# AuroraEchos/Sound-Event-Localization-and-Detection

Hardware: AMD Instinct MI355X
Metric: train-step samples/sec (8ch x 128mel x 512T) (higher is better)
Workload: dtype f32; 1 GPU; c3: DQSELD-TCN-S1-PHI_8ch train step, F=128 T=512 (U=L=192, SURVEY F3), batch 32/GPU, random-init weights; global_batch=32, parallelism=dp1, step_mode=graph (auto: probe 9.51 ms recorded / 10.23 ms eager per step), deterministic=True

## Files before the change

### sound-event-localization-and-detection_amd/csrc/first_stage.hip

```cpp
#include <string.h>
#include <type_traits>
#include "hc_common.h"

namespace seld {

constexpr int FS_K = 72;
constexpr int FS_KP = 80;
constexpr int FS_WEXT = 72, FS_DPAD = 4;
constexpr int FS_XR = 10;
constexpr int FS_NTILE = 15;

typedef unsigned int uintx4f __attribute__((ext_vector_type(4)));

__host__ __device__ constexpr int fs_tri(int t, int u) { return t * 5 - t * (t - 1) / 2 + (u - t); }

constexpr int FS_XI = (8 * FS_XR * (FS_WEXT / 4) + 255) / 256;
__device__ __forceinline__ void fs_load_x(const float* x, uintx4f (&v)[FS_XI], int n, int h0, int w0, int H, int W, int tid) {
    const unsigned S = (unsigned)(H * W);
    const unsigned OOB = 0xFFFFFFF0u;
    const __amdgpu_buffer_rsrc_t rsrc = __builtin_amdgcn_make_buffer_rsrc((void*)(x + (size_t)n * 8 * S), 0, 8u * S * 4u, 0x00020000);
    constexpr int qw = FS_WEXT / 4;
#pragma unroll
    for (int i = 0; i < FS_XI; ++i) {
        const int f = tid + 256 * i;
        const int row = f / qw, quad = f - row * qw;
        const int ch = row / FS_XR, xr = row - ch * FS_XR;
        const int hh = h0 - 1 + xr, ww = w0 - FS_DPAD + 4 * quad;
        const bool ok = f < 8 * FS_XR * qw && (unsigned)hh < (unsigned)H && (unsigned)ww < (unsigned)W;
        const unsigned e = ((unsigned)ch * (unsigned)H + (unsigned)hh) * (unsigned)W + (unsigned)ww;
        v[i] = __builtin_amdgcn_raw_buffer_load_b128(rsrc, ok ? e * 4u : OOB, 0, 0);
    }
}
__device__ __forceinline__ void fs_store_x(float* lds, const uintx4f (&v)[FS_XI], int tid) {
#pragma unroll
    for (int i = 0; i < FS_XI; ++i) {
        const int f = tid + 256 * i;
        if (f < 8 * FS_XR * (FS_WEXT / 4))
            *reinterpret_cast<float4*>(lds + f * 4) =
                make_float4(__uint_as_float(v[i][0]), __uint_as_float(v[i][1]), __uint_as_float(v[i][2]), __uint_as_float(v[i][3]));
    }
}
struct FsGramP {
    const float* x;
    float* part;
    int N, H, W;
    int nblocks;
};

__global__ __launch_bounds__(256, 2) void fs_gram_kernel(const FsGramP p) {
    __shared__ __attribute__((aligned(16))) float lds[8 * FS_XR * FS_WEXT > 3 * FS_NTILE * 256 ? 8 * FS_XR * FS_WEXT : 3 * FS_NTILE * 256];
    const int tid = threadIdx.x, lane = tid & 63;
    const int wave = __builtin_amdgcn_readfirstlane(tid >> 6);
    const int fr = lane & 15, fk = lane >> 4;
    int goff[5];
    float gone[5];
    bool gld[5];
#pragma unroll
    for (int t = 0; t < 5; ++t) {
        const int kk = 16 * t + fr;
        const int kc = kk < FS_K ? kk : 0;
        const int ch = kc / 9, tap = kc - ch * 9, kh = tap / 3, kw = tap - kh * 3;
        goff[t] = (ch * FS_XR + kh) * FS_WEXT + FS_DPAD + 16 * wave + fk + (kw - 1);
        gld[t] = kk < FS_K;
        gone[t] = kk == FS_K ? 1.f : 0.f;
    }
    floatx4 acc[FS_NTILE];
#pragma unroll
    for (int i = 0; i < FS_NTILE; ++i) acc[i] = (floatx4){0.f, 0.f, 0.f, 0.f};

    const int wq = p.W >> 6, hq = p.H >> 3;
    uintx4f xv[FS_XI];
    auto request = [&](int b) __attribute__((always_inline)) {
        const int n = b / (hq * wq), rem = b - n * (hq * wq);
        fs_load_x(p.x, xv, n, (rem / wq) * 8, (rem % wq) * 64, p.H, p.W, tid);
    };
    if ((int)blockIdx.x < p.nblocks) request(blockIdx.x);
    for (int b = blockIdx.x; b < p.nblocks; b += gridDim.x) {
        __syncthreads();
        fs_store_x(lds, xv, tid);
        __syncthreads();
        if (b + (int)gridDim.x < p.nblocks) request(b + gridDim.x);
        __builtin_amdgcn_sched_barrier(0);
#pragma unroll 1
        for (int r = 0; r < 8; ++r) {
#pragma unroll
            for (int j = 0; j < 4; ++j) {
                float v[5];
#pragma unroll
                for (int t = 0; t < 5; ++t) v[t] = gld[t] ? lds[goff[t] + r * FS_WEXT + 4 * j] : gone[t];
#pragma unroll
                for (int t = 0; t < 5; ++t)
#pragma unroll
                    for (int u = t; u < 5; ++u)
                        acc[fs_tri(t, u)] = __builtin_amdgcn_mfma_f32_16x16x4f32(v[t], v[u], acc[fs_tri(t, u)], 0, 0, 0);
            }
        }
    }
    __syncthreads();
    if (wave > 0) {
        float* dst = lds + (wave - 1) * FS_NTILE * 256 + lane * 4;
#pragma unroll
        for (int i = 0; i < FS_NTILE; ++i) *reinterpret_cast<floatx4*>(dst + i * 256) = acc[i];
    }
    __syncthreads();
    if (wave == 0) {
        float* out = p.part + (size_t)blockIdx.x * FS_NTILE * 256 + lane * 4;
#pragma unroll
        for (int i = 0; i < FS_NTILE; ++i) {
            floatx4 a = acc[i];
#pragma unroll
            for (int w = 0; w < 3; ++w) a += *reinterpret_cast<const floatx4*>(lds + w * FS_NTILE * 256 + i * 256 + lane * 4);
            *reinterpret_cast<floatx4*>(out + i * 256) = a;
        }
    }
}

__global__ __launch_bounds__(256) void fs_sum_parts_kernel(const float* __restrict__ part, int nparts, int n, double* __restrict__ red) {
    __shared__ double sh[4][64];
    const int lane = threadIdx.x & 63, wave = threadIdx.x >> 6;
    const int e = blockIdx.x * 64 + lane;
    double a = 0.0;
    if (e < n) {
        int w = wave;
        for (; w + 28 < nparts; w += 32) {
            float v[8];
#pragma unroll
            for (int k = 0; k < 8; ++k) v[k] = part[(size_t)(w + 4 * k) * n + e];
#pragma unroll
            for (int k = 0; k < 8; ++k) a += (double)v[k];
        }
        for (; w < nparts; w += 4) a += (double)part[(size_t)w * n + e];
    }
    sh[wave][lane] = a;
    __syncthreads();
    if (wave == 0 && e < n) red[e] = ((sh[0][lane] + sh[1][lane]) + sh[2][lane]) + sh[3][lane];
}
__global__ __launch_bounds__(256) void fs_gram_fold_kernel(const double* __restrict__ tiles, double* __restrict__ gram) {
    const int e = blockIdx.x * 256 + threadIdx.x;
    if (e >= FS_KP * FS_KP) return;
    const int i = e / FS_KP, j = e - i * FS_KP;
    const int lo = i < j ? i : j, hi = i < j ? j : i;
    const int t = lo >> 4, u = hi >> 4;
    int row, col;
    if (t == u) { row = i & 15; col = j & 15; }
    else { row = lo & 15; col = hi & 15; }
    const int ln = (row >> 2) * 16 + col;
    gram[e] = tiles[(size_t)fs_tri(t, u) * 256 + ln * 4 + (row & 3)];
}

struct FsW {
    const float* w[8];
    int A, OB, IB;
};
__device__ __forceinline__ float fs_wfull(const FsW& f, int c, int kk) {
    const int ch = kk / 9, tap = kk - ch * 9;
    const int po = c / f.OB, ob = c - po * f.OB;
    const int qi = ch / f.IB, ib = ch - qi * f.IB;
    float sign;
    const int comp = block_comp(f.A, po, qi, &sign);
    if (comp < 0) return 0.f;
    return sign * f.w[comp][((size_t)ob * f.IB + ib) * 9 + tap];
}

struct FsBnP {
    FsW w;
    const double* gram;
    const float* bias;
    float* mean;
    float* invstd;
    float* rmean;
    float* rvar;
    long long* nbt;
    float* wg;
    int C;
    float eps, momentum;
};
__global__ __launch_bounds__(256) void fs_bn_from_gram_kernel(const FsBnP p) {
    __shared__ double wrow[FS_K];
    __shared__ double red1[4], red2[4];
    const int c = blockIdx.x, tid = threadIdx.x;
    if (tid < FS_K) wrow[tid] = (double)fs_wfull(p.w, c, tid);
    __syncthreads();
    double m2 = 0.0, m1 = 0.0;
    if (tid < FS_K) {
        double row = 0.0;
        for (int k = 0; k < FS_K; ++k) row += wrow[k] * p.gram[tid * FS_KP + k];
        if (p.wg) p.wg[(size_t)c * FS_K + tid] = (float)row;
        m2 = wrow[tid] * row;
        m1 = wrow[tid] * p.gram[FS_K * FS_KP + tid];
    }
#pragma unroll
    for (int o = 32; o > 0; o >>= 1) {
        m1 += __shfl_xor(m1, o, 64);
        m2 += __shfl_xor(m2, o, 64);
    }
    if ((tid & 63) == 0) { red1[tid >> 6] = m1; red2[tid >> 6] = m2; }
    __syncthreads();
    if (tid != 0) return;
    if (c == 0 && p.nbt) *p.nbt += 1;
    const double count = p.gram[FS_K * FS_KP + FS_K];
    const double t1 = (red1[0] + red1[1] + red1[2] + red1[3]) / count;
    double var = (red2[0] + red2[1] + red2[2] + red2[3]) / count - t1 * t1;
    if (var < 0.0) var = 0.0;
    const double m = t1 + (p.bias ? (double)p.bias[c] : 0.0);
    p.mean[c] = (float)m;
    p.invstd[c] = (float)(1.0 / sqrt(var + (double)p.eps));
    if (p.rmean) p.rmean[c] = (1.f - p.momentum) * p.rmean[c] + p.momentum * (float)m;
    if (p.rvar) {
        const double unbiased = count > 1.0 ? var * count / (count - 1.0) : var;
        p.rvar[c] = (1.f - p.momentum) * p.rvar[c] + p.momentum * (float)unbiased;
    }
}

struct FsRedP {
    const float* dout;
    const float* out;
    const float* raw;
    const float* mean;
    const float* invstd;
    const float* gamma;
    const float* beta;
    float* part;
    int N, C, S;
    int nchunk;
    float scale;
};
__global__ __launch_bounds__(256) void fs_reduce_kernel(const FsRedP p) {
    const int c = blockIdx.y, chunk = blockIdx.x;
    const float mu = p.mean[c], is = p.invstd[c];
    const float ga = p.gamma[c], be = p.beta[c];
    const bool degenerate = ga == 0.f;
    const float inv_g = degenerate ? 0.f : 1.0f / ga, inv_scale = 1.0f / p.scale;
    const long long total = (long long)p.N * p.S;
    const long long per = ((total / 4 + p.nchunk - 1) / p.nchunk) * 4;
    const long long beg = (long long)chunk * per;
    long long end = beg + per;
    if (end > total) end = total;
    float v0 = 0.f, v1 = 0.f;
    for (long long k = beg + threadIdx.x * 4; k < end; k += 256 * 4) {
        const long long n = k / p.S;
        const size_t off = ((size_t)n * p.C + c) * p.S + (size_t)(k - n * p.S);
        float4 r4 = make_float4(0.f, 0.f, 0.f, 0.f);
        if (degenerate) r4 = *reinterpret_cast<const float4*>(p.raw + off);
        const float4 d4 = *reinterpret_cast<const float4*>(p.dout + off);
        const float4 o4 = *reinterpret_cast<const float4*>(p.out + off);
        const float rr[4] = {r4.x, r4.y, r4.z, r4.w}, dd[4] = {d4.x, d4.y, d4.z, d4.w}, oo[4] = {o4.x, o4.y, o4.z, o4.w};
#pragma unroll
        for (int e = 0; e < 4; ++e)
            if (oo[e] != 0.f) {
                const float dz = dd[e] * p.scale;
                v0 += dz * (degenerate ? (rr[e] - mu) * is : (oo[e] * inv_scale - be) * inv_g);
                v1 += dz;
            }
    }
    __shared__ float r0[4], r1[4];
    v0 = wave_sum(v0);
    v1 = wave_sum(v1);
    if ((threadIdx.x & 63) == 0) { r0[threadIdx.x >> 6] = v0; r1[threadIdx.x >> 6] = v1; }
    __syncthreads();
    if (threadIdx.x == 0) {
        float* o = p.part + ((size_t)c * p.nchunk + chunk) * 2;
        o[0] = (r0[0] + r0[1]) + (r0[2] + r0[3]);
        o[1] = (r1[0] + r1[1]) + (r1[2] + r1[3]);
    }
}
__global__ void fs_coef_kernel(const float* __restrict__ part, int nchunk, const float* __restrict__ mean,
                               const float* __restrict__ invstd, const float* __restrict__ gamma, int C, double count,
                               float* __restrict__ dgamma, float* __restrict__ dbeta, float* __restrict__ coef) {
    const int c = blockIdx.x * blockDim.x + threadIdx.x;
    if (c >= C) return;
    double s0 = 0.0, s1 = 0.0;
    for (int k = 0; k < nchunk; ++k) {
        s0 += (double)part[((size_t)c * nchunk + k) * 2];
        s1 += (double)part[((size_t)c * nchunk + k) * 2 + 1];
    }
    dgamma[c] += (float)s0;
    dbeta[c] += (float)s1;
    const float mu = mean[c], is = invstd[c], a = gamma[c] * is;
    const float k1 = (float)(s1 / count), k2 = (float)(s0 / count);
    coef[c] = -a * is * k2;
    coef[C + c] = a;
    coef[2 * C + c] = a * (mu * is * k2 - k1);
}

struct FsWgP {
    const float* x;
    const float* dout;
    const float* out;
    const unsigned char* idx;
    const float* invstd;
    const float* gamma;
    float* part;
    int N, C, H, W;
    int nblocks;
    float scale;
};

template <int NTW, bool DQ>
__global__ __launch_bounds__(512, 2) void fs_wgrad_kernel(const FsWgP p) {
    constexpr int NARROW = DQ ? NTW / 2 : 0;
    constexpr int NACC = NARROW * 3 + (NTW - NARROW) * 5;
    constexpr int XT = 8 * FS_XR * FS_WEXT;
    constexpr int RED = 2 * NACC * 256;
    __shared__ __attribute__((aligned(16))) float lds[(2 * XT > RED ? 2 * XT : RED) + 192];
    const int tid = threadIdx.x, lane = tid & 63;
    const int wave = __builtin_amdgcn_readfirstlane(tid >> 6);
    const int hc = wave >> 2, cq = wave & 3;
    const int fr = lane & 15, fk = lane >> 4;
    int goff[5];
    bool gld[5];
#pragma unroll
    for (int t = 0; t < 5; ++t) {
        const int kk = 16 * t + fr;
        const int kc = kk < FS_K ? kk : 0;
        const int ch = kc / 9, tap = kc - ch * 9, kh = tap / 3, kw = tap - kh * 3;
        goff[t] = (ch * FS_XR + kh) * FS_WEXT + FS_DPAD + 16 * cq + fk + (kw - 1);
        gld[t] = kk < FS_K;
    }
    auto ctile = [&](int i) __attribute__((always_inline)) -> int {
        if (DQ) return i < NARROW ? hc * NARROW + i : NTW + hc * NARROW + (i - NARROW);
        return hc * NTW + i;
    };
    float* const ab = lds + 2 * XT;
    for (int c = tid; c < p.C; c += 512) ab[c] = p.gamma[c] * p.invstd[c] * p.scale;
    auto acc_idx = [](int i, int u) constexpr { return i < NARROW ? i * 3 + u : NARROW * 3 + (i - NARROW) * 5 + u; };
    floatx4 acc[NACC];
#pragma unroll
    for (int i = 0; i < NACC; ++i) acc[i] = (floatx4){0.f, 0.f, 0.f, 0.f};

    const int wq = p.W >> 6, hq = p.H >> 3, PH = hq;
    const size_t PS = (size_t)PH * p.W;
    constexpr int QW = FS_WEXT / 4, NQ = 8 * FS_XR * QW, NST = (NQ + 511) / 512;
    float4 stage[NST];
    auto fetch_tile = [&](int b) __attribute__((always_inline)) {
        const int n = b / (hq * wq), rem = b - n * (hq * wq);
        const int h0 = (rem / wq) * 8, w0 = (rem % wq) * 64;
#pragma unroll
        for (int k = 0; k < NST; ++k) {
            const int f = tid + 512 * k;
            const int row = f / QW, quad = f - row * QW;
            const int ch = row / FS_XR, xr = row - ch * FS_XR;
            const int hh = h0 - 1 + xr, ww = w0 - FS_DPAD + 4 * quad;
            stage[k] = make_float4(0.f, 0.f, 0.f, 0.f);
            if (f < NQ && (unsigned)hh < (unsigned)p.H && (unsigned)ww < (unsigned)p.W)
                stage[k] = *reinterpret_cast<const float4*>(p.x + (((size_t)n * 8 + ch) * p.H + hh) * p.W + ww);
        }
    };
    auto store_tile = [&](float* buf) __attribute__((always_inline)) {
#pragma unroll
        for (int k = 0; k < NST; ++k) {
            const int f = tid + 512 * k;
            if (f < NQ) *reinterpret_cast<float4*>(buf + f * 4) = stage[k];
        }
    };
    float vz[NTW];
    unsigned rpk = 0;
    float ld_o[NTW], ld_d[NTW];
    unsigned ld_i[NTW];
    auto issue_group = [&](int b, int jg) __attribute__((always_inline)) {
        const int n = b / (hq * wq), rem = b - n * (hq * wq);
        const int q = rem / wq, w0 = (rem % wq) * 64;
#pragma unroll
        for (int i = 0; i < NTW; ++i) {
            const int chn = ctile(i) * 16 + fr;
            const size_t off = ((size_t)n * p.C + chn) * PS + (size_t)q * p.W + (size_t)(w0 + 16 * cq + 4 * jg + fk);
            ld_o[i] = p.out[off];
            ld_d[i] = p.dout[off];
            ld_i[i] = p.idx[off];
        }
    };
    auto finish_group = [&]() __attribute__((always_inline)) {
        unsigned pk = 0;
#pragma unroll
        for (int i = 0; i < NTW; ++i) {
            const float a_ = ab[ctile(i) * 16 + fr];
            vz[i] = ld_o[i] != 0.f ? ld_d[i] * a_ : 0.f;
            pk |= (ld_i[i] & 7u) << (3 * i);
        }
        rpk = pk;
    };
    int bufsel = 0;
    if ((int)blockIdx.x < p.nblocks) { fetch_tile(blockIdx.x); store_tile(lds); }
    __syncthreads();
    if ((int)blockIdx.x < p.nblocks) issue_group(blockIdx.x, 0);
    for (int b = blockIdx.x; b < p.nblocks; b += gridDim.x) {
        const float* xt = lds + bufsel * XT;
        const bool more = b + (int)gridDim.x < p.nblocks;
        if (more) fetch_tile(b + gridDim.x);
        float bv[5], bn_[5];
#pragma unroll
        for (int u = 0; u < 5; ++u) bv[u] = gld[u] ? xt[goff[u]] : 0.f;
#pragma unroll
        for (int jg = 0; jg < 4; ++jg) {
            finish_group();
            if (jg + 1 < 4) issue_group(b, jg + 1);
            else if (more) issue_group(b + gridDim.x, 0);
#pragma unroll 2
            for (int r = 0; r < 8; ++r) {
                const int rn = r + 1 < 8 ? r + 1 : 0, jn = r + 1 < 8 ? jg : (jg + 1 < 4 ? jg + 1 : 0);
#pragma unroll
                for (int u = 0; u < 5; ++u) bn_[u] = gld[u] ? xt[goff[u] + rn * FS_WEXT + 4 * jn] : 0.f;
#pragma unroll
                for (int i = 0; i < NTW; ++i) {
                    const float av = ((rpk >> (3 * i)) & 7u) == (unsigned)r ? vz[i] : 0.f;
#pragma unroll
                    for (int u = 0; u < (i < NARROW ? 3 : 5); ++u)
                        acc[acc_idx(i, u)] = __builtin_amdgcn_mfma_f32_16x16x4f32(av, bv[u], acc[acc_idx(i, u)], 0, 0, 0);
                }
#pragma unroll
                for (int u = 0; u < 5; ++u) bv[u] = bn_[u];
            }
        }
        if (more) store_tile(lds + (bufsel ^ 1) * XT);
        bufsel ^= 1;
        __syncthreads();
    }
#pragma unroll 1
    for (int k = 1; k < 4; ++k) {
        __syncthreads();
        if (cq == k) {
            float* dst = lds + hc * NACC * 256 + lane * 4;
#pragma unroll
            for (int i = 0; i < NACC; ++i) *reinterpret_cast<floatx4*>(dst + i * 256) = acc[i];
        }
        __syncthreads();
        if (cq == 0) {
            const float* src = lds + hc * NACC * 256 + lane * 4;
#pragma unroll
            for (int i = 0; i < NACC; ++i) acc[i] += *reinterpret_cast<const floatx4*>(src + i * 256);
        }
    }
    if (cq == 0) {
        float* out = p.part + (size_t)blockIdx.x * (2 * NTW) * 5 * 256 + lane * 4;
#pragma unroll
        for (int i = 0; i < NTW; ++i)
#pragma unroll
            for (int u = 0; u < 5; ++u) {
                floatx4 v = (floatx4){0.f, 0.f, 0.f, 0.f};
                if (u < (i < NARROW ? 3 : 5)) v = acc[acc_idx(i, u)];
                *reinterpret_cast<floatx4*>(out + (ctile(i) * 5 + u) * 256) = v;
            }
    }
}

struct FsWsumP {
    const double* sum;
    const float* wg;
    const double* gram;
    const float* coef;
    const float* bias;
    float* dwf;
    int C;
};
__global__ __launch_bounds__(256) void fs_wsum_kernel(const FsWsumP p) {
    const int e = blockIdx.x * 256 + threadIdx.x;
    if (e >= p.C * FS_K) return;
    const int c = e / FS_K, kk = e - c * FS_K;
    const int ct = c >> 4, row = c & 15, u = kk >> 4, col = kk & 15;
    double a = p.sum[((size_t)ct * 5 + u) * 256 + ((row >> 2) * 16 + col) * 4 + (row & 3)];
    const double sk = p.gram[FS_K * FS_KP + kk];
    a += (double)p.coef[c] * ((double)p.wg[e] + (p.bias ? (double)p.bias[c] * sk : 0.0)) + (double)p.coef[2 * p.C + c] * sk;
    p.dwf[e] = (float)a;
}
struct FsWfoldP {
    const float* dwf;
    float* dw[8];
    int A, OB, IB, C;
};
__global__ __launch_bounds__(256) void fs_wfold_kernel(const FsWfoldP p) {
    const int per = p.OB * p.IB * 9;
    const int e = blockIdx.x * 256 + threadIdx.x;
    if (e >= p.A * per) return;
    const int comp = e / per;
    int rem = e - comp * per;
    const int ob = rem / (p.IB * 9);
    rem -= ob * p.IB * 9;
    const int ib = rem / 9, tap = rem - ib * 9;
    float a = 0.f;
    for (int po = 0; po < p.A; ++po)
        for (int qi = 0; qi < p.A; ++qi) {
            float sign;
            if (block_comp(p.A, po, qi, &sign) != comp) continue;
            a += sign * p.dwf[(size_t)(po * p.OB + ob) * FS_K + (qi * p.IB + ib) * 9 + tap];
        }
    p.dw[comp][((size_t)ob * p.IB + ib) * 9 + tap] += a;
}

static int fs_shape_ok(const seld_conv_desc* d) {
    if (hc_validate(d) != SELD_OK) return 0;
    if (d->ndim != 2 || d->Cin != 8 || d->k[0] != 3 || d->k[1] != 3) return 0;
    if (d->stride[0] != 1 || d->stride[1] != 1 || d->dil[0] != 1 || d->dil[1] != 1 || d->pad[0] != 1 || d->pad[1] != 1) return 0;
    if (d->in[0] % 8 || d->in[1] % 64) return 0;
    if ((long long)d->N * d->Cout * d->in[0] * d->in[1] * 4 >= (1LL << 32)) return 0;
    return 1;
}
static int fs_gram_wgs(const seld_conv_desc* d) {
    const long long nblocks = (long long)d->N * (d->in[0] / 8) * (d->in[1] / 64);
    return (int)(nblocks < 512 ? nblocks : 512);
}

}
using namespace seld;

extern "C" size_t seld_first_stage_gram_workspace(const seld_conv_desc* d) {
    if (!fs_shape_ok(d)) return 0;
    return (size_t)FS_KP * FS_KP * sizeof(double) + (size_t)FS_NTILE * 256 * sizeof(double) +
           (size_t)fs_gram_wgs(d) * FS_NTILE * 256 * sizeof(float);
}

extern "C" int seld_first_stage_gram(const seld_conv_desc* d, const float* x, void* workspace, size_t workspace_bytes, void* stream) {
    if (!d || !x || !workspace) return SELD_EINVAL;
    const size_t need = seld_first_stage_gram_workspace(d);
    if (!need) return SELD_EUNSUPPORTED;
    if (workspace_bytes < need || ((uintptr_t)workspace & 15)) return SELD_EWORKSPACE;
    FsGramP p{};
    p.x = x; p.N = d->N; p.H = d->in[0]; p.W = d->in[1];
    p.nblocks = d->N * (d->in[0] / 8) * (d->in[1] / 64);
    double* gram = (double*)workspace;
    double* tiles = gram + FS_KP * FS_KP;
    p.part = (float*)(tiles + FS_NTILE * 256);
    const int nwg = fs_gram_wgs(d);
    hipStream_t st = (hipStream_t)stream;
    hipLaunchKernelGGL(fs_gram_kernel, dim3(nwg), dim3(256), 0, st, p);
    int rc = check_launch();
    if (rc) return rc;
    hipLaunchKernelGGL(fs_sum_parts_kernel, dim3(FS_NTILE * 256 / 64), dim3(256), 0, st, p.part, nwg, FS_NTILE * 256, tiles);
    rc = check_launch();
    if (rc) return rc;
    hipLaunchKernelGGL(fs_gram_fold_kernel, dim3((FS_KP * FS_KP + 255) / 256), dim3(256), 0, st, tiles, gram);
    return check_launch();
}

extern "C" int seld_first_stage_bn(const seld_conv_desc* d, const float* const w[8], const float* bias, const double* gram,
                                   float eps, float momentum, float* mean, float* invstd, float* running_mean,
                                   float* running_var, int64_t* num_batches_tracked, float* wg, void* stream) {
    if (!d || !w || !gram || !mean || !invstd) return SELD_EINVAL;
    if (!fs_shape_ok(d)) return SELD_EUNSUPPORTED;
    FsBnP p{};
    p.w.A = d->algebra; p.w.OB = d->Cout / d->algebra; p.w.IB = 8 / d->algebra;
    for (int i = 0; i < d->algebra; ++i) {
        if (!w[i]) return SELD_EINVAL;
        p.w.w[i] = w[i];
    }
    p.gram = gram; p.bias = bias; p.mean = mean; p.invstd = invstd; p.rmean = running_mean; p.rvar = running_var;
    p.nbt = (long long*)num_batches_tracked; p.wg = wg; p.C = d->Cout; p.eps = eps; p.momentum = momentum;
    hipLaunchKernelGGL(fs_bn_from_gram_kernel, dim3(d->Cout), dim3(256), 0, (hipStream_t)stream, p);
    return check_launch();
}

static int fs_wg_count(const seld_conv_desc* d) {
    const long long nblocks = (long long)d->N * (d->in[0] / 8) * (d->in[1] / 64);
    return (int)(nblocks < 256 ? nblocks : 256);
}
static int fs_red_chunks(const seld_conv_desc* d) {
    const long long total = (long long)d->N * (d->in[0] / 8) * d->in[1];
    long long n = total / 8192;
    if (n < 1) n = 1;
    if (n > 64) n = 64;
    return (int)n;
}

extern "C" size_t seld_first_stage_bwd_workspace(const seld_conv_desc* d) {
    if (!fs_shape_ok(d) || d->Cout % 64 || d->Cout > 192) return 0;
    if (d->algebra != 8 && d->Cout != 64) return 0;
    const int C = d->Cout;
    return (size_t)C * fs_red_chunks(d) * 2 * sizeof(float) + (size_t)3 * C * sizeof(float) + (size_t)C * FS_K * sizeof(float) +
           (size_t)(C / 16) * 5 * 256 * sizeof(double) + (size_t)fs_wg_count(d) * (C / 16) * 5 * 256 * sizeof(float) + 64;
}

extern "C" int seld_first_stage_bwd(const seld_conv_desc* d, const float* x, const float* dout, const float* out,
                                    const float* raw, const uint8_t* idx, const float* mean, const float* invstd, const float* gamma,
                                    const float* beta, const float* bias, const double* gram, const float* wg, float* dgamma, float* dbeta,
                                    float* const dw[8], float drop_p, void* workspace, size_t workspace_bytes, void* stream) {
    if (!d || !x || !dout || !out || !raw || !idx || !mean || !invstd || !gamma || !beta || !gram || !wg || !dgamma || !dbeta || !dw ||
        !workspace)
        return SELD_EINVAL;
    if (drop_p < 0.f || drop_p >= 1.f) return SELD_EINVAL;
    const size_t need = seld_first_stage_bwd_workspace(d);
    if (!need) return SELD_EUNSUPPORTED;
    if (workspace_bytes < need || ((uintptr_t)workspace & 15)) return SELD_EWORKSPACE;
    const int C = d->Cout, H = d->in[0], W = d->in[1], PH = H / 8;
    const int nchunk = fs_red_chunks(d), nwg = fs_wg_count(d);
    float* red_part = (float*)workspace;
    float* coef = red_part + (size_t)C * nchunk * 2;
    float* dwf = coef + 3 * C;
    double* wsumd = (double*)(((uintptr_t)(dwf + (size_t)C * FS_K) + 15) & ~(uintptr_t)15);
    float* part = (float*)(wsumd + (size_t)(C / 16) * 5 * 256);
    const float scale = 1.0f / (1.0f - drop_p);
    hipStream_t st = (hipStream_t)stream;

    FsRedP rp{};
    rp.dout = dout; rp.out = out; rp.raw = raw; rp.mean = mean; rp.invstd = invstd; rp.gamma = gamma; rp.beta = beta; rp.part = red_part;
    rp.N = d->N; rp.C = C; rp.S = PH * W; rp.nchunk = nchunk; rp.scale = scale;
    hipLaunchKernelGGL(fs_reduce_kernel, dim3(nchunk, C), dim3(256), 0, st, rp);
    int rc = check_launch();
    if (rc) return rc;
    hipLaunchKernelGGL(fs_coef_kernel, dim3((C + 255) / 256), dim3(256), 0, st, red_part, nchunk, mean, invstd, gamma, C,
                       (double)d->N * H * W, dgamma, dbeta, coef);
    rc = check_launch();
    if (rc) return rc;

    FsWgP wp{};
    wp.x = x; wp.dout = dout; wp.out = out; wp.idx = idx; wp.invstd = invstd; wp.gamma = gamma;
    wp.part = part; wp.N = d->N; wp.C = C; wp.H = H; wp.W = W; wp.nblocks = d->N * PH * (W / 64);
    wp.scale = scale;
    const bool dq = d->algebra == 8;
    if (C == 192) hipLaunchKernelGGL((fs_wgrad_kernel<6, true>), dim3(nwg), dim3(512), 0, st, wp);
    else if (C == 128) hipLaunchKernelGGL((fs_wgrad_kernel<4, true>), dim3(nwg), dim3(512), 0, st, wp);
    else { if (dq) hipLaunchKernelGGL((fs_wgrad_kernel<2, true>), dim3(nwg), dim3(512), 0, st, wp); else hipLaunchKernelGGL((fs_wgrad_kernel<2, false>), dim3(nwg), dim3(512), 0, st, wp); }
    rc = check_launch();
    if (rc) return rc;
    const int nsum = (C / 16) * 5 * 256;
    hipLaunchKernelGGL(fs_sum_parts_kernel, dim3(nsum / 64), dim3(256), 0, st, part, nwg, nsum, wsumd);
    rc = check_launch();
    if (rc) return rc;

    FsWsumP sp{};
    sp.sum = wsumd; sp.wg = wg; sp.gram = gram; sp.coef = coef; sp.bias = bias; sp.dwf = dwf; sp.C = C;
    hipLaunchKernelGGL(fs_wsum_kernel, dim3((C * FS_K + 255) / 256), dim3(256), 0, st, sp);
    rc = check_launch();
    if (rc) return rc;
    FsWfoldP fp{};
    fp.dwf = dwf; fp.A = d->algebra; fp.OB = C / d->algebra; fp.IB = 8 / d->algebra; fp.C = C;
    for (int i = 0; i < d->algebra; ++i) {
        if (!dw[i]) return SELD_EINVAL;
        fp.dw[i] = dw[i];
    }
    hipLaunchKernelGGL(fs_wfold_kernel, dim3((d->algebra * fp.OB * fp.IB * 9 + 255) / 256), dim3(256), 0, st, fp);
    return check_launch();
}
```

Baseline: 3649 samples/s.

## Use buffer-load-to-LDS DMA for x tiles and vectorized pooled-grad loads in wgrad

After: 3679 samples/s (median of 6 runs). About the same (+0.8%).

```diff
diff --git a/sound-event-localization-and-detection_amd/csrc/first_stage.hip b/sound-event-localization-and-detection_amd/csrc/first_stage.hip
--- a/sound-event-localization-and-detection_amd/csrc/first_stage.hip
+++ b/sound-event-localization-and-detection_amd/csrc/first_stage.hip
@@ -296,13 +296,21 @@
     float scale;
 };
 
+__device__ __forceinline__ void fs_dma16(unsigned lds_addr, unsigned voff, __amdgpu_buffer_rsrc_t rsrc) {
+    unsigned keep;
+    asm volatile("s_mov_b32 %0, m0\n\ts_mov_b32 m0, %1\n\ts_nop 0\n\tbuffer_load_dwordx4 %2, %3, 0 offen lds\n\ts_mov_b32 m0, %0"
+                 : "=&s"(keep) : "s"(lds_addr), "v"(voff), "s"(rsrc) : "memory");
+}
+
 template <int NTW, bool DQ>
 __global__ __launch_bounds__(512, 2) void fs_wgrad_kernel(const FsWgP p) {
     constexpr int NARROW = DQ ? NTW / 2 : 0;
     constexpr int NACC = NARROW * 3 + (NTW - NARROW) * 5;
     constexpr int XT = 8 * FS_XR * FS_WEXT;
     constexpr int RED = 2 * NACC * 256;
-    __shared__ __attribute__((aligned(16))) float lds[(2 * XT > RED ? 2 * XT : RED) + 192];
+    constexpr int XOFF = 2 * XT > RED ? 2 * XT : RED;
+    constexpr int NVW = NTW * 64 * 5;
+    __shared__ __attribute__((aligned(16))) float lds[XOFF + 192 + 8 * NVW];
     const int tid = threadIdx.x, lane = tid & 63;
     const int wave = __builtin_amdgcn_readfirstlane(tid >> 6);
     const int hc = wave >> 2, cq = wave & 3;
@@ -321,18 +329,30 @@
         if (DQ) return i < NARROW ? hc * NARROW + i : NTW + hc * NARROW + (i - NARROW);
         return hc * NTW + i;
     };
-    float* const ab = lds + 2 * XT;
+    float* const ab = lds + XOFF;
     for (int c = tid; c < p.C; c += 512) ab[c] = p.gamma[c] * p.invstd[c] * p.scale;
     auto acc_idx = [](int i, int u) constexpr { return i < NARROW ? i * 3 + u : NARROW * 3 + (i - NARROW) * 5 + u; };
     floatx4 acc[NACC];
 #pragma unroll
     for (int i = 0; i < NACC; ++i) acc[i] = (floatx4){0.f, 0.f, 0.f, 0.f};
 
-    const int wq = p.W >> 6, hq = p.H >> 3, PH = hq;
-    const size_t PS = (size_t)PH * p.W;
+    const int wq = p.W >> 6, hq = p.H >> 3;
+    const unsigned PS = (unsigned)hq * (unsigned)p.W;
+    const unsigned pelems = (unsigned)p.N * (unsigned)p.C * PS;
+    const __amdgpu_buffer_rsrc_t rs_out = __builtin_amdgcn_make_buffer_rsrc((void*)p.out, 0, pelems * 4u, 0x00020000);
+    const __amdgpu_buffer_rsrc_t rs_dout = __builtin_amdgcn_make_buffer_rsrc((void*)p.dout, 0, pelems * 4u, 0x00020000);
+    const __amdgpu_buffer_rsrc_t rs_idx = __builtin_amdgcn_make_buffer_rsrc((void*)p.idx, 0, pelems, 0x00020000);
+    const unsigned lane_e = (unsigned)fr * PS + (unsigned)(16 * cq + 4 * fk);
+    auto blk_e = [&](int b) __attribute__((always_inline)) -> unsigned {
+        const int n = b / (hq * wq), rem = b - n * (hq * wq);
+        return (unsigned)n * (unsigned)p.C * PS + (unsigned)(rem / wq) * (unsigned)p.W + (unsigned)((rem % wq) * 64);
+    };
+
     constexpr int QW = FS_WEXT / 4, NQ = 8 * FS_XR * QW, NST = (NQ + 511) / 512;
-    float4 stage[NST];
-    auto fetch_tile = [&](int b) __attribute__((always_inline)) {
+    const __amdgpu_buffer_rsrc_t rs_x =
+        __builtin_amdgcn_make_buffer_rsrc((void*)p.x, 0, (unsigned)p.N * 8u * (unsigned)p.H * (unsigned)p.W * 4u, 0x00020000);
+    const unsigned lds0 = (unsigned)(size_t)(__attribute__((address_space(3))) unsigned char*)lds;
+    auto dma_tile = [&](int b, int buf) __attribute__((always_inline)) {
         const int n = b / (hq * wq), rem = b - n * (hq * wq);
         const int h0 = (rem / wq) * 8, w0 = (rem % wq) * 64;
 #pragma unroll
@@ -341,60 +361,86 @@
             const int row = f / QW, quad = f - row * QW;
             const int ch = row / FS_XR, xr = row - ch * FS_XR;
             const int hh = h0 - 1 + xr, ww = w0 - FS_DPAD + 4 * quad;
-            stage[k] = make_float4(0.f, 0.f, 0.f, 0.f);
-            if (f < NQ && (unsigned)hh < (unsigned)p.H && (unsigned)ww < (unsigned)p.W)
-                stage[k] = *reinterpret_cast<const float4*>(p.x + (((size_t)n * 8 + ch) * p.H + hh) * p.W + ww);
+            const bool ok = (unsigned)hh < (unsigned)p.H && (unsigned)ww < (unsigned)p.W;
+            const unsigned e = (((unsigned)n * 8u + (unsigned)ch) * (unsigned)p.H + (unsigned)hh) * (unsigned)p.W + (unsigned)ww;
+            if (f < NQ)
+                fs_dma16(lds0 + ((unsigned)buf * XT + (unsigned)(512 * k + 64 * wave) * 4u) * 4u, ok ? e * 4u : 0xFFFFFFF0u, rs_x);
         }
     };
-    auto store_tile = [&](float* buf) __attribute__((always_inline)) {
-#pragma unroll
-        for (int k = 0; k < NST; ++k) {
-            const int f = tid + 512 * k;
-            if (f < NQ) *reinterpret_cast<float4*>(buf + f * 4) = stage[k];
-        }
+
+    float cvz[NTW][4];
+    unsigned cix[NTW];
+    uintx4f ld_o[NTW], ld_d[NTW];
+    unsigned ld_i[NTW];
+    float* const nv = lds + XOFF + 192 + wave * NVW;
+    auto issue = [&](unsigned be, int i) __attribute__((always_inline)) {
+        const unsigned e = be + (unsigned)ctile(i) * 16u * PS;
+        ld_o[i] = __builtin_amdgcn_raw_buffer_load_b128(rs_out, lane_e * 4u, e * 4u, 0);
+        ld_d[i] = __builtin_amdgcn_raw_buffer_load_b128(rs_dout, lane_e * 4u, e * 4u, 0);
+        ld_i[i] = __builtin_amdgcn_raw_buffer_load_b32(rs_idx, lane_e, e, 0);
     };
-    float vz[NTW];
-    unsigned rpk = 0;
-    float ld_o[NTW], ld_d[NTW];
-    unsigned ld_i[NTW];
-    auto issue_group = [&](int b, int jg) __attribute__((always_inline)) {
-        const int n = b / (hq * wq), rem = b - n * (hq * wq);
-        const int q = rem / wq, w0 = (rem % wq) * 64;
+    auto convert = [&](int i) __attribute__((always_inline)) {
+        const float a_ = ab[ctile(i) * 16 + fr];
+        float z[4];
+#pragma unroll
+        for (int e = 0; e < 4; ++e) z[e] = __uint_as_float(ld_o[i][e]) != 0.f ? __uint_as_float(ld_d[i][e]) * a_ : 0.f;
+        *reinterpret_cast<float4*>(nv + (i * 64 + lane) * 4) = make_float4(z[0], z[1], z[2], z[3]);
+        reinterpret_cast<unsigned*>(nv)[NTW * 256 + i * 64 + lane] = ld_i[i];
+    };
+    auto take_next = [&]() __attribute__((always_inline)) {
+        __builtin_amdgcn_fence(__ATOMIC_RELEASE, "wavefront");
+        __builtin_amdgcn_wave_barrier();
+        __builtin_amdgcn_fence(__ATOMIC_ACQUIRE, "wavefront");
+        const unsigned char* const nb = reinterpret_cast<const unsigned char*>(nv + NTW * 256);
 #pragma unroll
         for (int i = 0; i < NTW; ++i) {
-            const int chn = ctile(i) * 16 + fr;
-            const size_t off = ((size_t)n * p.C + chn) * PS + (size_t)q * p.W + (size_t)(w0 + 16 * cq + 4 * jg + fk);
-            ld_o[i] = p.out[off];
-            ld_d[i] = p.dout[off];
-            ld_i[i] = p.idx[off];
+            unsigned pk = 0;
+#pragma unroll
+            for (int jg = 0; jg < 4; ++jg) {
+                cvz[i][jg] = nv[(i * 64 + jg * 16 + fr) * 4 + fk];
+                pk |= (unsigned)nb[(i * 64 + jg * 16 + fr) * 4 + fk] << (8 * jg);
+            }
+            cix[i] = pk;
         }
     };
-    auto finish_group = [&]() __attribute__((always_inline)) {
-        unsigned pk = 0;
-#pragma unroll
-        for (int i = 0; i < NTW; ++i) {
-            const float a_ = ab[ctile(i) * 16 + fr];
-            vz[i] = ld_o[i] != 0.f ? ld_d[i] * a_ : 0.f;
-            pk |= (ld_i[i] & 7u) << (3 * i);
-        }
-        rpk = pk;
-    };
+    auto issue_at = [](int i) constexpr { return 1 + (3 * i) / NTW; };
+
     int bufsel = 0;
-    if ((int)blockIdx.x < p.nblocks) { fetch_tile(blockIdx.x); store_tile(lds); }
+    if ((int)blockIdx.x < p.nblocks) {
+        dma_tile(blockIdx.x, 0);
+        const unsigned be = blk_e(blockIdx.x);
+#pragma unroll
+        for (int i = 0; i < NTW; ++i) issue(be, i);
+    }
+    asm volatile("s_waitcnt vmcnt(0)" ::: "memory");
     __syncthreads();
-    if ((int)blockIdx.x < p.nblocks) issue_group(blockIdx.x, 0);
+    if ((int)blockIdx.x < p.nblocks) {
+#pragma unroll
+        for (int i = 0; i < NTW; ++i) convert(i);
+    }
+    take_next();
     for (int b = blockIdx.x; b < p.nblocks; b += gridDim.x) {
         const float* xt = lds + bufsel * XT;
         const bool more = b + (int)gridDim.x < p.nblocks;
-        if (more) fetch_tile(b + gridDim.x);
+        const unsigned be_next = more ? blk_e(b + gridDim.x) : 0u;
+        if (more) dma_tile(b + gridDim.x, bufsel ^ 1);
         float bv[5], bn_[5];
 #pragma unroll
         for (int u = 0; u < 5; ++u) bv[u] = gld[u] ? xt[goff[u]] : 0.f;
 #pragma unroll
         for (int jg = 0; jg < 4; ++jg) {
-            finish_group();
-            if (jg + 1 < 4) issue_group(b, jg + 1);
-            else if (more) issue_group(b + gridDim.x, 0);
+            if (more) {
+#pragma unroll
+                for (int i = 0; i < NTW; ++i)
+                    if (issue_at(i) + 1 == jg) convert(i);
+#pragma unroll
+                for (int i = 0; i < NTW; ++i)
+                    if (issue_at(i) == jg) issue(be_next, i);
+            }
+            unsigned rpk = 0;
+#pragma unroll
+            for (int i = 0; i < NTW; ++i) rpk |= ((cix[i] >> (8 * jg)) & 7u) << (3 * i);
+            __builtin_amdgcn_sched_barrier(0);
 #pragma unroll 2
             for (int r = 0; r < 8; ++r) {
                 const int rn = r + 1 < 8 ? r + 1 : 0, jn = r + 1 < 8 ? jg : (jg + 1 < 4 ? jg + 1 : 0);
@@ -402,7 +448,7 @@
                 for (int u = 0; u < 5; ++u) bn_[u] = gld[u] ? xt[goff[u] + rn * FS_WEXT + 4 * jn] : 0.f;
 #pragma unroll
                 for (int i = 0; i < NTW; ++i) {
-                    const float av = ((rpk >> (3 * i)) & 7u) == (unsigned)r ? vz[i] : 0.f;
+                    const float av = ((rpk >> (3 * i)) & 7u) == (unsigned)r ? cvz[i][jg] : 0.f;
 #pragma unroll
                     for (int u = 0; u < (i < NARROW ? 3 : 5); ++u)
                         acc[acc_idx(i, u)] = __builtin_amdgcn_mfma_f32_16x16x4f32(av, bv[u], acc[acc_idx(i, u)], 0, 0, 0);
@@ -411,8 +457,14 @@
                 for (int u = 0; u < 5; ++u) bv[u] = bn_[u];
             }
         }
-        if (more) store_tile(lds + (bufsel ^ 1) * XT);
+        if (more) {
+#pragma unroll
+            for (int i = 0; i < NTW; ++i)
+                if (issue_at(i) == 3) convert(i);
+            take_next();
+        }
         bufsel ^= 1;
+        asm volatile("s_waitcnt vmcnt(0)" ::: "memory");
         __syncthreads();
     }
 #pragma unroll 1
```
